# ielym/fastvision

Hardware: AMD Instinct MI355X
Metric: images/sec (640×640, bs=32/GPU) YOLOv3 train step, 1/2/4/8 MI355X (higher is better)
Workload: dtype bf16

## Files before the change

### fastvision_amd/_lib.py

```python
import ctypes as C
import os

HERE = os.path.dirname(os.path.abspath(__file__))
LIB_PATH = os.path.join(HERE, 'csrc', 'libfastvision_amd.so')
if os.environ.get('FVA_LIB_PATH'):
    if os.environ.get('FVA_EXPERIMENTS') == '1':
        LIB_PATH = os.environ['FVA_LIB_PATH']
        import sys
        print(f'fastvision_amd: EXPERIMENT -- loading {LIB_PATH} instead of the in-tree library (FVA_LIB_PATH)', file=sys.stderr)
    else:
        raise RuntimeError('fastvision_amd: FVA_LIB_PATH is set but FVA_EXPERIMENTS=1 is not -- refusing to load another library silently')

F32, BF16 = 0, 1


class ConvDesc(C.Structure):
    _fields_ = [(n, C.c_int32) for n in ('dtype', 'B', 'H', 'W', 'Cin', 'Cout', 'ksize', 'stride', 'in_pad', 'dy_pad')]


class GConvDesc(C.Structure):
    _fields_ = [(n, C.c_int32) for n in ('dtype', 'B', 'H', 'W', 'C', 'groups', 'stride', 'in_pad', 'dy_pad')]


class HeadLevel(C.Structure):
# ... 60 lines not shown
class ColourJob(C.Structure):
    _fields_ = [(n, C.c_int32) for n in ('h', 'w', 'clahe', 'hsv', 'blur')] + [('perm', C.c_int32 * 3)]


class MatchOut(C.Structure):
    _fields_ = [(n, C.c_void_p) for n in ('count', 'b', 'gx', 'gy', 'a', 'cls', 'xywh', 'anc')]


_P, _I, _L, _F = C.c_void_p, C.c_int32, C.c_int64, C.c_float
_D = C.POINTER(ConvDesc)
_H = C.POINTER(HeadLevel)
_G = C.POINTER(GConvDesc)

PROTOTYPES = {
    'fva_last_error': (C.c_char_p, []),
    'fva_version': (_I, []),
    'fva_profile_start': (_I, [_I]),
    'fva_profile_classes': (_I, [C.c_uint32, _I]),
    'fva_side_stream_fork': (_I, [_P, C.POINTER(C.c_void_p)]),
    'fva_side_stream_join': (_I, [_P]),
    'fva_side_stream_renew': (_I, []),
    'fva_conv_debug_stamps': (_I, [_P, _I]),
    'fva_conv_patch_kernel': (_I, [_I]),
    'fva_profile_stop': (_I, [_P, _P, _P, _I]),
    'fva_conv_pack_weights': (_I, [_D, _P, _P, _P, _P]),
    'fva_conv_packed_elems': (_L, [_D, _I]),
    'fva_conv_pack_weights_multi': (_I, [_P, _I, _L, _P]),
    'fva_conv_pack_weights_tiled': (_I, [_P, _I, _I, _P]),
    'fva_conv_last_kernel': (C.c_char_p, []),
    'fva_conv_fwd': (_I, [_D, _P, _P, _P, _P, _P]),
    'fva_conv1x1_fwd_apply': (_I, [_D, _P, _P, _P, _P, _I, _P, _P, _P, _P, _P]),
    'fva_conv_fwd_acc': (_I, [_D, _P, _P, _P, _P, _I, _P]),
    'fva_bn_acc_finalize': (_I, [C.POINTER(BnFwdAcc), _L, _I, _P]),
    'fva_bn_silu_apply_acc': (_I, [_I, _P, C.POINTER(BnFwdAcc), _P, _I, _P, _I, _I, _I, _I, _I, _P]),
    'fva_conv1x1_fwd_apply_acc': (_I, [_D, _P, C.POINTER(BnFwdAcc), _P, _I, _P, _P, _P, _P, _I, _P]),
    'fva_conv_fwd_bnact': (_I, [_D, _P, _P, _P, _P, _P, _P, _I, _P]),
    'fva_conv_stat_blocks': (_I, [_D]),
    'fva_conv_dgrad': (_I, [_D, _P, _P, _P, _P, _P]),
    'fva_conv_dgrad_bnstats': (_I, [_D, _P, _P, _P, _P, C.POINTER(BnBwdFuse), _P]),
    'fva_conv_dgrad_stat_rows': (_I, [_D]),
    'fva_conv_wgrad': (_I, [_D, _P, _P, _P, _I, _P, _L, _P]),
    'fva_conv_wgrad_workspace': (_L, [_D]),
    'fva_conv_wgrad_plan': (_I, [_I]),
    'fva_stem_fwd': (_I, [_I, _P, _P, _P, _P, _P, _L, _I, _I, _I, _I, _I, _P]),
    'fva_stem_fwd_workspace': (_L, [_I, _I, _I, _I]),
    'fva_stem_stat_blocks': (_I, [_I, _I, _I, _I]),
# ... 86 lines not shown
    'fva_bn_frozen_bwd_blocks': (_I, [_I, _I, _I, _I, _I, _I]),
    'fva_bn_silu_frozen_bwd': (_I, [_I, _P, _P, _P, _P, _P, _P, _P, _P, _I, _I, _I, _I, _I, _P]),
    'fva_bn_relu_frozen_bwd': (_I, [_I, _P, _P, _P, _P, _P, _P, _P, _P, _I, _I, _I, _I, _I, _P]),
    'fva_bn_frozen_bwd_finalize': (_I, [_P, _I, _I, _I, _P, _P, _P, _P, _P]),
    'fva_bn_frozen_stats': (_I, [_I, _P, _P, _P, _F, _P, _P, _P]),
    'fva_stem7_kp': (_I, [_I, _I]),
    'fva_stem7_patches': (_I, [_I, _P, _P, _I, _I, _I, _I, _P]),
    'fva_maxpool3s2_fwd': (_I, [_I, _P, _I, _P, _I, _I, _I, _I, _I, _P]),
    'fva_maxpool3s2_bwd': (_I, [_I, _P, _P, _I, _P, _I, _I, _I, _I, _P]),
    'fva_subsample2_fwd': (_I, [_I, _P, _I, _P, _I, _I, _I, _I, _P]),
    'fva_subsample2_bwd': (_I, [_I, _P, _P, _I, _I, _I, _I, _P]),
    'fva_bn_add_relu_apply': (_I, [_I, _P, _P, _P, _P, _I, _P, _P, _P, _P, _I, _I, _I, _I, _I, _P]),
    'fva_bn_add_relu_bwd_blocks': (_I, [_I, _L, _I]),
    'fva_bn_add_relu_bwd_reduce': (_I, [_I, _P, _P, _P, _P, _P, _P, _P, _I, _P, _P, _P, _P, _P, _P, _P, _I, _I, _I, _I, _I, _P]),
    'fva_bn_add_relu_bwd_apply': (_I, [_I, _P, _P, _P, _P, _P, _P, _P, _P, _I, _P, _P, _P, _P, _P, _P, _P, _P, _I, _P, _I, _I, _I, _I, _P]),
    'fva_gconv_fwd': (_I, [_G, _P, _P, _P, _P, _P]),
    'fva_gconv_stat_blocks': (_I, [_G]),
    'fva_gconv_dgrad': (_I, [_G, _P, _P, _P, _P]),
    'fva_gconv_wgrad': (_I, [_G, _P, _P, _P, _P, _L, _P]),
    'fva_gconv_wgrad_workspace': (_L, [_G]),
}
LABEL_I64, LABEL_F32 = 0, 1
REDUCE_MEAN, REDUCE_SUM = 0, 1
UNCHECKED = {'fva_conv_patch_kernel', 'fva_sgd_chunk_elems', 'fva_ema_chunk_elems', 'fva_rows_relu_bwd_rows', 'fva_colour_workspace', 'fva_conv_dgrad_stat_rows', 'fva_bias_relu_bwd_rows', 'fva_colsum_scratch_rows', 'fva_last_error', 'fva_version', 'fva_profile_stop', 'fva_conv_last_kernel', 'fva_conv_packed_elems', 'fva_conv_stat_blocks', 'fva_conv_wgrad_workspace', 'fva_conv_wgrad_plan',
             'fva_stem_stat_blocks', 'fva_stem_fused_blocks', 'fva_stem_wgrad_workspace', 'fva_stem_fwd_workspace', 'fva_stem_wgrad_mfma_workspace', 'fva_bn_bwd_blocks', 'fva_bn_partial_rows', 'fva_yolov3_loss_workspace',
             'fva_demo_loss_workspace', 'fva_demo_ciou_loss_workspace', 'fva_nms_candidates_workspace', 'fva_nms_select_workspace', 'fva_softmax_ce_workspace', 'fva_bn_frozen_bwd_blocks', 'fva_stem7_kp', 'fva_bn_add_relu_bwd_blocks', 'fva_gconv_stat_blocks', 'fva_gconv_wgrad_workspace'}

_lib = None


def load():
    global _lib
    if _lib is not None:
        return _lib
    if not os.path.exists(LIB_PATH):
        raise RuntimeError(f'fastvision_amd: {LIB_PATH} is missing -- the HIP extension is REQUIRED (no CPU fallback). '
                           'Build it with `python fastvision_amd/csrc/build.py`.')
    lib = C.CDLL(LIB_PATH)
    for name, (res, args) in PROTOTYPES.items():
        fn = getattr(lib, name)
        fn.restype, fn.argtypes = res, args
    _lib = lib
    return lib


tracer = None

# ... 22 lines not shown
```

### fastvision_amd/csrc/conv_igemm.hip

```cpp
#include <stddef.h>
#include <stdlib.h>

#include "common.h"

namespace {

enum { EPI_STATS = 0, EPI_PLAIN = 1, EPI_HEAD = 2, EPI_BNACT = 3, EPI_BNB = 4 };
constexpr int MAX_TAPS = 10;

struct IgemmParams {
    const void* in;
    const void* wt;
    void* out;
    float* stats;
    int acc_rep, bnb_rep, ax_rep;
    long long* stats_acc;
    const float* bias;
    const float* scale;
    int act;
    const float* shift;
    int M, N, C;
    int OW, OHW;
    FastDiv div_ow, div_ohw;
    int in_img, in_row;
    int sy, sx, y0, x0;
    int ktiles, kt_per_tap, halfrow;
    int ktaps;
    int tap_pix[MAX_TAPS];
    int tap_w[MAX_TAPS];
    int out_dense;
    int out_img, out_row, osy, osx, ooy, oox, out_pitch;
    const void* addend;
    int nblocks;
    const void* bnb_y;
    const float *bnb_scale, *bnb_shift, *bnb_mean, *bnb_rstd;
    float* bnb_part;
    long long* bnb_acc;
    int bnb_row0, bnb_C;
    const void* ax_y;
    const void* ax_res;
    void* ax_z;
    const float *ax_scale, *ax_shift;
    int ax_pad, ax_res_pad, ax_H, ax_W;
    long long* ax_acc;
    long long* ax_zero;
    const float *ax_gamma, *ax_beta;
    float *ax_rm, *ax_rv;
    long long* ax_nbt;
    float ax_momentum, ax_eps;
    BnN ax_n;
    float *ax_save_mean, *ax_save_rstd, *ax_scale_out, *ax_shift_out;
    long long* stamps;
    int stamp_rows;
    int pt_tx, pt_ty, pt_H, pt_W;
    int pt_tiles, pt_tpb;
    FastDiv pt_div_tx, pt_div_img;
// ... 177 lines not shown
#pragma unroll
    for (int mt = 0; mt < 4; ++mt)
#pragma unroll
        for (int nt = 0; nt < 4; ++nt)
#pragma unroll
            for (int j = 0; j < 4; ++j) f(mt * 16 + r, nt * 16 + g * 4 + j, nt, acc.a[mt][nt][j]);
}
template <typename F>
__device__ __forceinline__ void foreach_acc(Acc<float>& acc, int lane, F&& f) {
    const int r = lane & 31, h = lane >> 5;
#pragma unroll
    for (int mt = 0; mt < 2; ++mt)
#pragma unroll
        for (int nt = 0; nt < 2; ++nt)
#pragma unroll
            for (int e = 0; e < 16; ++e) f(mt * 32 + (e & 3) + 8 * (e >> 2) + 4 * h, nt * 32 + r, nt, acc.a[mt][nt][e]);
}

template <int N>
__device__ __forceinline__ void wait_vmcnt() {
    asm volatile("s_waitcnt vmcnt(%0)" ::"n"(N) : "memory");
}

template <typename T, int BM, int BN, int EPI, int NSTAGE, bool AX = false>
__global__ __launch_bounds__((BM / 64) * (BN / 64) * 64) void igemm_kernel(const IgemmParams p) {
    static_assert(!AX || (sizeof(T) == 2 && EPI == EPI_STATS), "the produced-operand form is the bf16 training forward of a 1x1 layer");
    constexpr int EPC = 16 / (int)sizeof(T);
    constexpr int BK = 8 * EPC;
    constexpr int WN = BN / 64;
    constexpr int NW = (BM / 64) * WN;
    constexpr int NT = NW * 64;
    static_assert(NW % 2 == 0, "the source swizzle assumes an even wave count");
    constexpr int A_BYTES = BM * 128, B_BYTES = BN * 128, STAGE = A_BYTES + B_BYTES;
    constexpr int A_ITERS = BM / (8 * NW), B_ITERS = BN / (8 * NW);
    constexpr bool IS_BF16 = sizeof(T) == 2;
    extern __shared__ __attribute__((aligned(16))) char smem[];

    const int tid = threadIdx.x, lane = tid & 63, w = tid >> 6;
    const int wr = w / WN, wc = w % WN;
    auto stamp = [&](int i) {
        if (p.stamps && tid == 0 && (int)blockIdx.x < p.stamp_rows) p.stamps[(int64_t)blockIdx.x * 8 + i] = wall_clock64();
    };
    stamp(0);

    const int nwg = gridDim.x, bid = blockIdx.x;
    const int xcd = bid & 7, xq = nwg >> 3, xr = nwg & 7;
    const int logical = (xcd < xr ? xcd * (xq + 1) : xr * (xq + 1) + (xcd - xr) * xq) + (bid >> 3);
    const int mblk = logical / p.nblocks, nblk = logical - mblk * p.nblocks;
    const int m0 = mblk * BM, n0 = nblk * BN;

    const T* a_ptr[A_ITERS];
    const T* b_ptr[B_ITERS];
    const int lrow = lane >> 3;
    const int sw = ((w & 1) << 2) + (lane >> 4);
    const int chunk = (lane & 7) ^ sw;
    const int tapsel = chunk >> 2;
    const int sub = p.halfrow ? (chunk & 3) : chunk;
#pragma unroll
    for (int i = 0; i < A_ITERS; ++i) {
        int m = m0 + (i * NW + w) * 8 + lrow;
        m = m < p.M ? m : p.M - 1;
        const uint32_t b = fd_div((uint32_t)m, p.div_ohw);
        const uint32_t rem = (uint32_t)m - b * (uint32_t)p.OHW;
        const uint32_t oy = fd_div(rem, p.div_ow);
        const uint32_t ox = rem - oy * (uint32_t)p.OW;
        const int64_t pix = (int64_t)b * p.in_img + (int64_t)(oy * p.sy + p.y0) * p.in_row + (ox * p.sx + p.x0);
        a_ptr[i] = (const T*)p.in + pix * p.C + sub * EPC;
    }
#pragma unroll
    for (int i = 0; i < B_ITERS; ++i) {
        int n = n0 + (i * NW + w) * 8 + lrow;
        n = n < p.N ? n : p.N - 1;
        b_ptr[i] = (const T*)p.wt + (int64_t)n * p.C + sub * EPC;
    }

    constexpr bool USE_KTAB = BN >= 128;
    constexpr int COEF_BYTES = (EPI == EPI_BNB && IS_BF16 && BN >= 128) ? 4 * BN * 4 : 0;
    float* coef_tab = (float*)(smem + NSTAGE * STAGE);
    int* ktab = (int*)(smem + NSTAGE * STAGE + COEF_BYTES);
    constexpr int COEF_PER_THREAD = COEF_BYTES > 0 ? 4 * BN / NT : 0;
    float coef_v[COEF_PER_THREAD > 0 ? COEF_PER_THREAD : 1];
    if constexpr (COEF_BYTES > 0) {
#pragma unroll
        for (int j = 0; j < COEF_PER_THREAD; ++j) coef_v[j] = bnb_coef_at<BN, NT>(p, tid + j * NT, n0);
    }
    if constexpr (USE_KTAB) {
        const int nent = p.halfrow ? 2 * p.ktiles : p.ktiles;
        for (int e = tid; e < nent; e += NT) {
            int t, kk;
            if (p.halfrow) { t = e; kk = 0; }
            else if (p.ktaps) { kk = e / p.ktaps; t = e - kk * p.ktaps; }
            else { t = e / p.kt_per_tap; kk = e - t * p.kt_per_tap; }
            int tp = 0, tw = 0;
#pragma unroll
            for (int i = 0; i < MAX_TAPS; ++i)
                if (i == t) { tp = p.tap_pix[i]; tw = p.tap_w[i]; }
            ktab[2 * e] = tp * p.C + kk * BK;
            ktab[2 * e + 1] = tw * p.N * p.C + kk * BK;
        }
        __syncthreads();
    }
    stamp(6);
    int ld_tap = 0, ld_kk = 0;
    auto load_tile = [&](int kt, int stage) {
        char* sA = smem + stage * STAGE;
        char* sB = sA + A_BYTES;
        int aoff, boff;
        if constexpr (USE_KTAB) {
            const int e = p.halfrow ? 2 * kt + tapsel : kt;
            aoff = ktab[2 * e];
            boff = ktab[2 * e + 1];
        } else {
            const int t = p.halfrow ? ld_tap + tapsel : ld_tap;
            int tp = 0, tw = 0;
#pragma unroll
// ... 10 lines not shown
#pragma unroll
        for (int i = 0; i < B_ITERS; ++i)
            __builtin_amdgcn_global_load_lds(GLB_PTR(b_ptr[i] + boff), LDS_PTR(sB + (i * NW + w) * 1024), 16, 0, 0);
    };

    bf16x8 y_pre[8], a_pre[8];
    constexpr bool PREFETCH = (EPI == EPI_BNB || EPI == EPI_PLAIN) && sizeof(T) == 2;
    if constexpr (PREFETCH) {
        constexpr int CPR = BN / 8, RSTEP = NT / CPR;
        static_assert(BM * CPR / NT == 8, "the prefetch covers the whole store loop");
        const int cc = tid % CPR, r0 = tid / CPR;
        const int n = n0 + cc * 8;
#pragma unroll
        for (int j = 0; j < 8; ++j) {
            const int m = m0 + r0 + j * RSTEP;
            int64_t oi = 0;
            if (n < p.N && m < p.M) {
                int64_t pixel = m;
                if (!p.out_dense) {
                    const uint32_t b = fd_div((uint32_t)m, p.div_ohw);
                    const uint32_t rem = (uint32_t)m - b * (uint32_t)p.OHW;
                    const uint32_t oy = fd_div(rem, p.div_ow);
                    const uint32_t ox = rem - oy * (uint32_t)p.OW;
                    pixel = (int64_t)b * p.out_img + (int64_t)(oy * p.osy + p.ooy) * p.out_row + (ox * p.osx + p.oox);
                }
                oi = pixel * p.out_pitch + n;
            }
            if constexpr (EPI == EPI_BNB) y_pre[j] = ld_stream((const bf16_t*)p.bnb_y + oi);
            if (p.addend != nullptr) a_pre[j] = ld_stream((const bf16_t*)p.addend + oi);
        }
    }

    Acc<T> acc;
    if constexpr (sizeof(T) == 2) {
#pragma unroll
        for (int i = 0; i < 4; ++i)
#pragma unroll
            for (int j = 0; j < 4; ++j) acc.a[i][j] = f32x4{0.f, 0.f, 0.f, 0.f};
    } else {
#pragma unroll
        for (int i = 0; i < 2; ++i)
#pragma unroll
            for (int j = 0; j < 2; ++j)
#pragma unroll
                for (int e = 0; e < 16; ++e) acc.a[i][j][e] = 0.f;
    }

// ... 131 lines not shown
            m = live ? m : p.M - 1;
            const uint32_t b = fd_div((uint32_t)m, p.div_ohw);
            const uint32_t rem = (uint32_t)m - b * (uint32_t)p.OHW;
            const uint32_t oy = fd_div(rem, p.div_ow);
            const uint32_t ox = rem - oy * (uint32_t)p.OW;
            ax_yo[i] = (uint32_t)m * (uint32_t)p.C + chunk * 8;
            ax_zo[i] = (b * zHW + (oy + zp) * zW + ox + zp) * (uint32_t)p.C + chunk * 8;
            ax_ro[i] = (b * rHW + (oy + rp) * rW + ox + rp) * (uint32_t)p.C + chunk * 8;
            ax_fl[i] = (live ? 1u : 0u) | (zp > 0 && live ? ((ox == 0 ? 2u : 0u) | (ox == (uint32_t)p.ax_W - 1 ? 4u : 0u) | (oy == 0 ? 8u : 0u) |
                                                           (oy == (uint32_t)p.ax_H - 1 ? 16u : 0u)) : 0u);
        }
        ax_load_raw(0, std::integral_constant<int, 0>{});
        if constexpr (AXT) {
            for (int c = tid; c < p.C; c += NT) ax_coef(c, logical == 0, ax_tab[c], ax_tab[p.C + c]);
            __syncthreads();
        }
        if (AXT && p.ax_acc != nullptr && logical == 0) {
            if (tid == 0 && p.ax_nbt) *p.ax_nbt += 1;
            fx_zero(p.ax_zero, p.C, p.ax_rep, tid, NT);
        }
        ax_issue_b(0, 0);
    } else {
        load_tile(0, 0);
        if (p.ktiles > 1) load_tile(1, 1);
    }
    stamp(1);
    for (int kt = 0; kt < p.ktiles; ++kt) {
        if constexpr (AX) {
            if (AXS == 1 || (kt & 1) == 0) ax_step(kt, std::integral_constant<int, 0>{});
            else ax_step(kt, std::integral_constant<int, AXS - 1>{});
            if (kt == 0) stamp(2);
        } else {
        if (kt == 0 && p.ktiles > 1) wait_vmcnt<LPT>();
        else wait_vmcnt<0>();
        __builtin_amdgcn_s_barrier();
        if (kt == 0) stamp(2);
        if (kt >= 1 && kt + 1 < p.ktiles) load_tile(kt + 1, st_cur ^ 1);
        }
        const char* sA = smem + st_cur * STAGE;
        const char* sB = sA + A_BYTES;
        st_cur ^= 1;
        if constexpr (IS_BF16) {
            const int r = lane & 15, g = lane >> 4, sr = (r >> 1) & 7;
            const char* pa = sA + (wr * 64 + r) * 128;
            const char* pb = sB + (wc * 64 + r) * 128;
#pragma unroll
            for (int ks = 0; ks < 2; ++ks) {
                const int co = ((ks * 4 + g) ^ sr) << 4;
                bf16x8 af[4], bfr[4];
#pragma unroll
                for (int t = 0; t < 4; ++t) {
                    af[t] = *(const bf16x8*)(pa + t * 16 * 128 + co);
                    bfr[t] = *(const bf16x8*)(pb + t * 16 * 128 + co);
                }
#pragma unroll
                for (int mt = 0; mt < 4; ++mt)
#pragma unroll
                    for (int nt = 0; nt < 4; ++nt)
                        acc.a[mt][nt] = __builtin_amdgcn_mfma_f32_16x16x32_bf16(bfr[nt], af[mt], acc.a[mt][nt], 0, 0, 0);
            }
// ... 95 lines not shown
                }
                __syncthreads();
                if (w < BN / 32) {
                    const int which = lane >> 5, col = w * 32 + (lane & 31);
                    float s = 0.f;
#pragma unroll
                    for (int k = 0; k < WMc; ++k) s += red[(which * WMc + k) * BN + col];
                    if (n0 + col < p.N) {
                        if (p.stats_acc != nullptr) fx_atomic_add(fx_replica(p.stats_acc, p.N, p.acc_rep), p.N, which, n0 + col, s);
                        else *(p.stats + ((int64_t)mblk * 2 + which) * p.N + n0 + col) = s;
                    }
                }
                __syncthreads();
            }
        }
    }

    auto out_pixel = [&](int m) -> int64_t {
        if (p.out_dense) return m;
        const uint32_t b = fd_div((uint32_t)m, p.div_ohw);
        const uint32_t rem = (uint32_t)m - b * (uint32_t)p.OHW;
        const uint32_t oy = fd_div(rem, p.div_ow);
        const uint32_t ox = rem - oy * (uint32_t)p.OW;
        return (int64_t)b * p.out_img + (int64_t)(oy * p.osy + p.ooy) * p.out_row + (ox * p.osx + p.oox);
    };

    if constexpr (EPI == EPI_HEAD) {
        float* out = (float*)p.out;
        foreach_acc(acc, lane, [&](int row, int col, int, float v) {
            const int m = m0 + wrow0 + row, n = n0 + wcol0 + col;
            if (m < p.M && n < p.N) out[(int64_t)m * p.out_pitch + n] = v + p.bias[n];
        });
    } else if constexpr (!IS_BF16) {
        float* out = (float*)p.out;
        int64_t pix_cache = -1;
        int m_cache = -1;
        constexpr bool bnb = EPI == EPI_BNB;
        float b1[2] = {0.f, 0.f}, b2[2] = {0.f, 0.f}, ksc[2], ksh[2], kmu[2], krs[2];
        if constexpr (bnb) {
#pragma unroll
            for (int nt = 0; nt < 2; ++nt) {
                int c = n0 + wcol0 + nt * 32 + (lane & 31);
                c = c < p.N ? c : p.N - 1;
                c = c >= p.bnb_C ? c - p.bnb_C : c;
                ksc[nt] = p.bnb_scale[c]; ksh[nt] = p.bnb_shift[c]; kmu[nt] = p.bnb_mean[c]; krs[nt] = p.bnb_rstd[c];
            }
        }
// ... 54 lines not shown
            static_assert(4 * BN <= NT || EPI != EPI_BNB || COEF_BYTES > 0, "one table entry per thread");
            if (tid < 4 * BN) coef_v[0] = bnb_coef_at<BN, NT>(p, tid, n0);
        }
        {
            const int r = lane & 15, g = lane >> 4;
#pragma unroll
            for (int mt = 0; mt < 4; ++mt)
#pragma unroll
                for (int nt = 0; nt < 4; ++nt) {
                    f32x4 v = acc.a[mt][nt];
                    const int col = wcol0 + nt * 16 + 4 * g;
                    if constexpr (EPI == EPI_BNACT) {
#pragma unroll
                        for (int j = 0; j < 4; ++j) v[j] = bnact_f(p, v[j], n0 + col + j < p.N ? n0 + col + j : p.N - 1);
                    }
                    *(u32x2*)(smem + (wrow0 + mt * 16 + r) * PITCH + col * 2) = u32x2{cvt_pk_bf16(v[0], v[1]), cvt_pk_bf16(v[2], v[3])};
                }
        }
        if constexpr (EPI == EPI_BNB && COEF_BYTES == 0) {
            if (tid < 4 * BN) coef_tab[tid] = coef_v[0];
        }
        __syncthreads();
        stamp(4);
        store_tile_bf16<EPI, BM, BN, NT, PITCH>(p, smem, tid, n0, mblk, [&](int row) { const int m = m0 + row; return m < p.M ? out_pixel(m) : (int64_t)-1; },
                                                EPI == EPI_BNB ? y_pre : nullptr, PREFETCH ? a_pre : nullptr, coef_tab);
    }
    stamp(5);
}

template <typename T, int BM, int BN, int EPI, int NSTAGE, bool AX = false>
int launch_one(const IgemmParams& p, hipStream_t s) {
    const int mblocks = cdiv(p.M, BM);
    IgemmParams q = p;
    q.nblocks = cdiv(p.N, BN);
    static const bool stamp_tiles = [] { const char* e = getenv("FVA_STAMP_IGEMM"); return e && atoi(e) != 0; }();
    q.stamps = stamp_tiles ? fva_debug_stamps_ptr() : nullptr;
    q.stamp_rows = stamp_tiles ? fva_debug_stamps_rows() : 0;
    constexpr int KTAB_MAX = 16384;
    const int nent = (p.halfrow ? 2 : 1) * p.ktiles;
    if (BN >= 128 && nent * 8 > KTAB_MAX) return fva_fail(FVA_ERR_ARG, "igemm: %d k-tiles exceed the offset table (%d)", p.ktiles, KTAB_MAX / 8);
    const int ktab_bytes = BN >= 128 ? (nent * 8 > 4096 ? (nent * 8 + 255) & ~255 : 4096) : 0;
    constexpr int coef_bytes = (EPI == EPI_BNB && sizeof(T) == 2 && BN >= 128) ? 4 * BN * 4 : 0;
    const int smem = NSTAGE * (BM + BN) * 128 + ktab_bytes + coef_bytes;
    static bool attr_done = false;
    if (!attr_done) {
        (void)hipFuncSetAttribute((const void*)igemm_kernel<T, BM, BN, EPI, NSTAGE, AX>, hipFuncAttributeMaxDynamicSharedMemorySize,
                                  NSTAGE * (BM + BN) * 128 + (BN >= 128 ? KTAB_MAX : 0) + coef_bytes);
        attr_done = true;
    }
    hipLaunchKernelGGL((igemm_kernel<T, BM, BN, EPI, NSTAGE, AX>), dim3(mblocks * q.nblocks), dim3((BM / 64) * (BN / 64) * 64), smem, s, q);
    FVA_LAUNCH_CHECK("igemm_kernel");
    fva_note_kernel(AX ? (BM == 128 ? "igemm128ax" : "igemm256x64ax") : (BM == 128 ? "igemm128" : "igemm256x64"));
    return FVA_OK;
}

// ... 322 lines not shown
#define FVA_EPI_STAMPS 0
#endif
template <int EPI>
__global__ __launch_bounds__(512) void igemm8_kernel(const IgemmParams p, const Igemm8Diag sk) {
    constexpr int MT = 8;
    constexpr int WM = 16 * MT;
    constexpr int BM = 2 * WM, BN = 256, NT = 512, BK = 64;
    constexpr int HALF = 128 * 128, BUF = 4 * HALF;
    constexpr int EPI_BYTES = BM * (BN * 2 + 16);
    constexpr int TAB0 = EPI_BYTES > 2 * BUF ? EPI_BYTES : 2 * BUF;
    extern __shared__ __attribute__((aligned(16))) char smem[];
    const int tid = threadIdx.x, lane = tid & 63, w = tid >> 6;
    const int wr = w >> 2, wc = w & 3;
    auto stamp = [&](int i) {
        if (sk.stamps && tid == 0 && (int)blockIdx.x < sk.stamp_rows) {
            sk.stamps[(int64_t)blockIdx.x * 8 + i] = wall_clock64();
            sk.stamps[(int64_t)blockIdx.x * 8 + 4 + i] = clock64();
        }
    };
#if !FVA_EPI_STAMPS
    stamp(0);
#endif

    const int nwg = gridDim.x, bid = blockIdx.x;
    const int xcd = bid & 7, xq = nwg >> 3, xr = nwg & 7;
    const int logical = (xcd < xr ? xcd * (xq + 1) : xr * (xq + 1) + (xcd - xr) * xq) + (bid >> 3);
    const int KT = p.ktiles;

    int* ktab = (int*)(smem + TAB0);
    for (int e = tid; e < KT; e += NT) {
        int t, kk;
        if (p.ktaps) { kk = e / p.ktaps; t = e - kk * p.ktaps; }
        else { t = e / p.kt_per_tap; kk = e - t * p.kt_per_tap; }
        int tp = 0, tw = 0;
#pragma unroll
        for (int i = 0; i < MAX_TAPS; ++i)
            if (i == t) { tp = p.tap_pix[i]; tw = p.tap_w[i]; }
        ktab[2 * e] = tp * p.C + kk * BK;
        ktab[2 * e + 1] = tw * p.N * p.C + kk * BK;
    }

    const int lrow = lane >> 3;
    const int chunk = (lane & 7) ^ (((w & 1) << 2) + (lane >> 4));
    const int r = lane & 15, g = lane >> 4, sr = (r >> 1) & 7;
    const int co0 = (g ^ sr) << 4, co1 = ((4 + g) ^ sr) << 4;
    const int a_row = (wr * 64 + r) * 128, b_row = (wc * 32 + r) * 128;

    {
        const int tile = logical, kt0 = 0, kt1 = KT;
        const int mblk = tile / p.nblocks, nblk = tile - mblk * p.nblocks;
        const int m0 = mblk * BM, n0 = nblk * BN;
        __syncthreads();
        float* coef_tab = (float*)(smem + TAB0 + 4096);
        if constexpr (EPI == EPI_BNB) bnb_fill_lds<BN, NT>(p, coef_tab, tid, n0);

        uint32_t a_off[2][2], b_off[2][2];
// ... 156 lines not shown
                    *(f32x4*)(red + ((1 * 2 + wr_e) * 16 + r_e) * RP + col_e + ni * 16) = s2[ni];
                }
                __syncthreads();
                {
                    const int which = lane_e >> 5, col = (tid_e >> 6) * 32 + (lane_e & 31);
                    float s = 0.f;
#pragma unroll
                    for (int i = 0; i < 32; ++i) s += red[(which * 32 + i) * RP + col];
                    if (n0 + col < p.N) {
                        if (p.stats_acc != nullptr) fx_atomic_add(fx_replica(p.stats_acc, p.N, p.acc_rep), p.N, which, n0 + col, s);
                        else *(p.stats + ((int64_t)mblk * 2 + which) * p.N + n0 + col) = s;
                    }
                }
                __syncthreads();
            }
        }

        auto out_pixel = [&](int m) -> int64_t {
            if (p.out_dense) return m;
            const uint32_t b = fd_div((uint32_t)m, p.div_ohw);
            const uint32_t rem = (uint32_t)m - b * (uint32_t)p.OHW;
            const uint32_t oy = fd_div(rem, p.div_ow);
            const uint32_t ox = rem - oy * (uint32_t)p.OW;
            return (int64_t)b * p.out_img + (int64_t)(oy * p.osy + p.ooy) * p.out_row + (ox * p.osx + p.oox);
        };
        constexpr int PITCH = BN * 2 + 16;
#if FVA_EPI_STAMPS
        stamp(1);
#endif
#pragma unroll
        for (int mi = 0; mi < MT; ++mi)
#pragma unroll
            for (int ni = 0; ni < 4; ++ni) {
                f32x4 v = acc[mi][ni];
                if constexpr (EPI == EPI_BNACT) {
#pragma unroll
                    for (int j = 0; j < 4; ++j) v[j] = bnact_f(p, v[j], n0 + col_e + ni * 16 + j);
                }
                *(u32x2*)(smem + (row_e + mi * 16) * PITCH + (col_e + ni * 16) * 2) = u32x2{cvt_pk_bf16(v[0], v[1]), cvt_pk_bf16(v[2], v[3])};
            }
        __syncthreads();
#if FVA_EPI_STAMPS
        stamp(2);
#endif
        store_tile_bf16<EPI, BM, BN, NT, PITCH>(p, smem, tid_e, n0, mblk, [&](int row) { const int m = m0 + row; return m < p.M ? out_pixel(m) : (int64_t)-1; },
                                                nullptr, nullptr, EPI == EPI_BNB ? coef_tab : nullptr);
    }
    stamp(3);
}

constexpr int IGEMM8_SMEM = 256 * (256 * 2 + 16) + 4096 + 4096;

inline bool igemm8_enabled() {
    static bool v = [] {
        const char* e = getenv("FVA_IGEMM8");
        return !e || atoi(e) != 0;
    }();
    return v;
}
inline bool use_igemm8(int dtype, int64_t M, int N, int C, int ntaps, int64_t in_pixels) {
    if (!igemm8_enabled() || dtype != FVA_BF16 || N % 256 || C % 64) return false;
    if (in_pixels * C * 2 >= (1ll << 31) || (int64_t)(ntaps + 1) * N * C * 2 >= (1ll << 31)) return false;
    const int64_t ktiles = (int64_t)ntaps * (C / 64), tiles = (int64_t)cdiv(M, 256) * (N / 256);
    if (ktiles > 496 || ktiles < 8) return false;
    if (tiles < 128) return false;
    static const int min_kt = [] { const char* e = getenv("FVA_IGEMM8_MINKT"); return e ? atoi(e) : 16; }();
    return ktiles >= min_kt || tiles <= 256;
}

long long* g_stamps = nullptr;
int g_stamp_rows = 0;

template <int EPI>
int launch_igemm8(const IgemmParams& p, hipStream_t s) {
    IgemmParams q = p;
    q.nblocks = p.N / 256;
    const int tiles = cdiv(p.M, 256) * q.nblocks;
    static bool attr_done = false;
    if (!attr_done) {
        (void)hipFuncSetAttribute((const void*)igemm8_kernel<EPI>, hipFuncAttributeMaxDynamicSharedMemorySize, IGEMM8_SMEM);
        attr_done = true;
    }
    Igemm8Diag sk{};
    sk.stamps = g_stamps;
    sk.stamp_rows = g_stamp_rows;
    hipLaunchKernelGGL((igemm8_kernel<EPI>), dim3(tiles), dim3(512), IGEMM8_SMEM, s, q, sk);
    fva_note_kernel("igemm8");
    FVA_LAUNCH_CHECK("igemm8_kernel");
    return FVA_OK;
}

inline bool wide_tile(int N) { return N >= 128; }

enum { IGEMM_128, IGEMM_256x64, IGEMM_8PHASE };
struct IgemmChoice {
    int kernel, bm;
};
inline IgemmChoice choose_igemm(int dtype, int64_t M, int N, int C, int ntaps, int64_t in_pixels, bool halfrow, bool head) {
    if (!head && !halfrow && use_igemm8(dtype, M, N, C, ntaps, in_pixels)) return {IGEMM_8PHASE, 256};
    return wide_tile(N) ? IgemmChoice{IGEMM_128, 128} : IgemmChoice{IGEMM_256x64, 256};
// ... 198 lines not shown
}
inline bool dgrad_paired(int dtype, int ksize, int stride, int Cin, int Cout) {
    return ksize == 3 && stride == 2 && Cin <= pair_max_cin() && !use_pdgrad2(dtype, ksize, stride, Cout, Cin);
}

int packed_taps(const fva_conv_desc* d, int for_dgrad) {
    if (for_dgrad && dgrad_paired(d->dtype, d->ksize, d->stride, d->Cin, d->Cout)) return 12;

    const int kk = d->ksize * d->ksize;
    const int C = for_dgrad ? d->Cout : d->Cin;
    return (halfrow_mode(d->dtype, C) && (kk & 1)) ? kk + 1 : kk;
}

enum { LAUNCH_IGEMM, LAUNCH_PATCH1, LAUNCH_PATCH2 };
struct ConvLaunch {
    int kind;
    IgemmChoice igemm;
    int64_t M;
    int N, OH, OW;
    int ntaps, tap_pix[MAX_TAPS], tap_w[MAX_TAPS];
    int ostep, ooy, oox;
    int row_blocks;
    int rows_per_block;
};

void set_grid(ConvLaunch& e, int B, int OH, int OW, int N) {
    e.M = (int64_t)B * OH * OW; e.N = N; e.OH = OH; e.OW = OW;
    e.ntaps = 0; e.ostep = 1; e.ooy = e.oox = 0; e.rows_per_block = 1;
}
void add_tap(ConvLaunch& e, int pix, int w) { e.tap_pix[e.ntaps] = pix; e.tap_w[e.ntaps] = w; ++e.ntaps; }
void close_taps(ConvLaunch& e, int zero_tap) { e.tap_w[e.ntaps] = zero_tap; }
void finish_igemm(ConvLaunch& e, int dtype, int C, int64_t in_pixels, bool head) {
    e.kind = LAUNCH_IGEMM;
    e.igemm = choose_igemm(dtype, e.M, e.N, C, e.ntaps, in_pixels, halfrow_mode(dtype, C), head);
    e.row_blocks = cdiv(e.M, e.igemm.bm);
}
template <typename G>
void finish_patch(ConvLaunch& e, int kind, const fva_conv_desc* d) {
    e.kind = kind;
    e.row_blocks = patch_tiles<G>(d->B, d->H, d->W);
}

ConvLaunch fwd_plan(const fva_conv_desc* d, int epi) {
    const int k = d->ksize, s = d->stride, in_row = d->W + 2 * d->in_pad, in_img = (d->H + 2 * d->in_pad) * in_row;
    ConvLaunch e;
    set_grid(e, d->B, (d->H - 1) / s + 1, (d->W - 1) / s + 1, d->Cout);
    if (k * k < MAX_TAPS) {
        for (int kh = 0; kh < k; ++kh)
            for (int kw = 0; kw < k; ++kw) add_tap(e, kh * in_row + kw, kh * k + kw);
        close_taps(e, k * k);
    } else {
        e.ntaps = k * k;
    }
    finish_igemm(e, d->dtype, d->Cin, (int64_t)(d->B + 1) * in_img, epi == EPI_HEAD);
    if (epi == EPI_STATS && use_pconv(d->dtype, k, s, d->Cin, d->Cout, d->H, d->W)) finish_patch<PconvGeom>(e, LAUNCH_PATCH1, d);
    return e;
}

int parity_taps(int parity, int kh[2], int off[2]) {
    if (parity == 0) { kh[0] = 1; off[0] = 0; return 1; }
    kh[0] = 0; off[0] = 1; kh[1] = 2; off[1] = 0;
    return 2;
}

int dgrad_plan(const fva_conv_desc* d, ConvLaunch out[4]) {
    const int k = d->ksize, s = d->stride, pd = k / 2, dtype = d->dtype;
    const int OH = (d->H - 1) / s + 1, OW = (d->W - 1) / s + 1, in_row = OW + 2 * d->dy_pad;
    const int64_t in_pixels = (int64_t)(d->B + 1) * (OH + 2 * d->dy_pad) * in_row;
    ConvLaunch& e = out[0];
    if (s == 1) {
        set_grid(e, d->B, d->H, d->W, d->Cin);
        for (int kh = 0; kh < k; ++kh)
            for (int kw = 0; kw < k; ++kw) add_tap(e, (2 * pd - kh) * in_row + (2 * pd - kw), kh * k + kw);
        close_taps(e, k * k);
        finish_igemm(e, dtype, d->Cout, in_pixels, false);
        if (use_pconv(dtype, k, s, d->Cout, d->Cin, d->H, d->W)) finish_patch<PconvGeom>(e, LAUNCH_PATCH1, d);
        return 1;
    }
    if (use_pdgrad2(dtype, k, s, d->Cout, d->Cin)) {
        set_grid(e, d->B, d->H, d->W, d->Cin);
        finish_patch<Pdgrad2Geom>(e, LAUNCH_PATCH2, d);
        return 1;
    }
    const bool paired = dgrad_paired(dtype, k, s, d->Cin, d->Cout);
    int n = 0;
    for (int py = 0; py < 2; ++py)
        for (int px = 0; px < (paired ? 1 : 2); ++px) {
            ConvLaunch& q = out[n++];
            set_grid(q, d->B, d->H / 2, d->W / 2, paired ? 2 * d->Cin : d->Cin);
            int ky[2], yo[2], kx[2] = {0, 1}, xo[2] = {0, 1};
            const int ny = parity_taps(py, ky, yo), nx = paired ? 2 : parity_taps(px, kx, xo);
            for (int a = 0; a < ny; ++a)
                for (int b = 0; b < nx; ++b) add_tap(q, (d->dy_pad + yo[a]) * in_row + d->dy_pad + xo[b], ky[a] * (paired ? 2 : 3) + kx[b]);
            q.ostep = 2; q.ooy = py; q.oox = px;
            q.rows_per_block = paired ? 2 : 1;
            close_taps(q, paired ? 0 : 9);
            finish_igemm(q, dtype, d->Cout, in_pixels, false);
        }
    return n;
}

}

long long* fva_debug_stamps_ptr() { return g_stamps; }
int fva_debug_stamps_rows() { return g_stamp_rows; }
extern "C" {

int fva_conv_patch_kernel(int on) {
    const int prev = pconv_enabled() ? 1 : 0;
    g_pconv = on ? 1 : 0;
    return prev;
}

int fva_conv_debug_stamps(void* stamps, int32_t rows) {
    if (stamps && rows < 1) return fva_fail(FVA_ERR_ARG, "fva_conv_debug_stamps: rows must be >= 1");
    g_stamps = (long long*)stamps;
    g_stamp_rows = stamps ? rows : 0;
    return FVA_OK;
}

int64_t fva_conv_packed_elems(const fva_conv_desc* d, int for_dgrad) {
    if (!d) return 0;
    return (int64_t)packed_taps(d, for_dgrad) * d->Cout * d->Cin;
}

int fva_conv_pack_weights(const fva_conv_desc* d, const float* w, void* w_fwd, void* w_dgrad, void* stream) {
    int rc = check_desc(d, "fva_conv_pack_weights");
    if (rc) return rc;
    if (!w) return fva_fail(FVA_ERR_ARG, "fva_conv_pack_weights: null weights");
    const int paired = dgrad_paired(d->dtype, d->ksize, d->stride, d->Cin, d->Cout) ? 1 : 0;
    const int tf = packed_taps(d, 0), td = paired ? d->ksize * d->ksize : packed_taps(d, 1);
    const int64_t total = (int64_t)(tf > td ? tf : td) * d->Cout * d->Cin;
    const int grid = (int)((total + 255) / 256 < 4096 ? (total + 255) / 256 : 4096);
// ... 18 lines not shown
    hipLaunchKernelGGL(pack_weights_tiled_kernel, dim3(total_tiles), dim3(256), 0, (hipStream_t)stream, table_dev, n);
    FVA_LAUNCH_CHECK("pack_weights_tiled_kernel");
    return FVA_OK;
}

int32_t fva_conv_stat_blocks(const fva_conv_desc* d) {
    if (!d) return 0;
    return fwd_plan(d, EPI_STATS).row_blocks;
}

static void set_launch(IgemmParams& p, const ConvLaunch& e, int dtype) {
    p.M = (int)e.M;
    p.N = e.N;
    p.OW = e.OW;
    p.OHW = e.OH * e.OW;
    p.div_ow = make_fastdiv(p.OW);
    p.div_ohw = make_fastdiv(p.OHW);
    for (int t = 0; t < e.ntaps; ++t) {
        p.tap_pix[t] = e.tap_pix[t];
        p.tap_w[t] = e.tap_w[t];
    }
    p.tap_w[e.ntaps] = e.tap_w[e.ntaps];
    finish_taps(p, e.ntaps, dtype);
    p.out_dense = e.ostep == 1 ? 1 : 0;
    if (!p.out_dense) {
        p.osy = p.osx = e.ostep;
        p.ooy = e.ooy;
        p.oox = e.oox;
    }
}

static int setup_fwd(const fva_conv_desc* d, int epi, IgemmParams& p, ConvLaunch& e, const char* who) {
    int rc = check_desc(d, who);
    if (rc) return rc;
    rc = check_red_channels(d->dtype, d->Cin, who);
    if (rc) return rc;
    e = fwd_plan(d, epi);
    p = IgemmParams();
    p.acc_rep = p.bnb_rep = p.ax_rep = 1;
    p.C = d->Cin;
    p.in_row = d->W + 2 * d->in_pad;
    p.in_img = (d->H + 2 * d->in_pad) * p.in_row;
    p.sy = p.sx = d->stride;
    p.y0 = p.x0 = d->in_pad - d->ksize / 2;
    set_launch(p, e, d->dtype);
    p.out_pitch = d->Cout;
// ... 214 lines not shown
```

### include/fastvision_amd.h

```cpp
#ifndef FASTVISION_AMD_H
#define FASTVISION_AMD_H

#include <stdint.h>

#ifdef __cplusplus
extern "C" {
#endif

typedef enum { FVA_F32 = 0, FVA_BF16 = 1 } fva_dtype;

typedef enum {
    FVA_OK = 0,
    FVA_ERR_ARG = -1,
    FVA_ERR_LAUNCH = -2,
    FVA_ERR_WORKSPACE = -3
} fva_status;

const char* fva_last_error(void);
int fva_version(void);

int fva_profile_start(int32_t max_spans);
int fva_profile_classes(uint32_t mask, int32_t stride);

int fva_side_stream_fork(void* main_stream, void** side_stream);
// ... 7 lines not shown
    int32_t Cin, Cout;
    int32_t ksize, stride;
    int32_t in_pad;
    int32_t dy_pad;
} fva_conv_desc;

int fva_conv_pack_weights(const fva_conv_desc* d, const float* w_oihw, void* w_fwd, void* w_dgrad, void* stream);
int64_t fva_conv_packed_elems(const fva_conv_desc* d, int for_dgrad);
typedef struct {
    const float* w;
    void* w_fwd;
    void* w_dgrad;
    int32_t Cout, Cin, ksize, taps_fwd, taps_dgrad, dtype;
    int32_t dgrad_paired;
    int32_t tile_start;
} fva_pack_entry;
int fva_conv_pack_weights_multi(const fva_pack_entry* table, int32_t n, int64_t max_elems, void* stream);
int fva_conv_pack_weights_tiled(const fva_pack_entry* table, int32_t n, int32_t total_tiles, void* stream);

const char* fva_conv_last_kernel(void);

int fva_conv_debug_stamps(void* stamps, int32_t rows);
int fva_conv_patch_kernel(int on);

int fva_conv_fwd(const fva_conv_desc* d, const void* x, const void* w_fwd, void* y, float* stats_partial, void* stream);
int fva_conv1x1_fwd_apply(const fva_conv_desc* d, const void* y_prev, const float* scale, const float* shift, const void* residual,
                          int32_t res_pad, void* z, const void* w_fwd, void* y, float* stats_partial, void* stream);
int fva_conv_fwd_bnact(const fva_conv_desc* d, const void* x, const void* w_fwd, const float* scale, const float* shift,
                       const void* residual, void* z, int32_t z_pad, void* stream);
int32_t fva_conv_stat_blocks(const fva_conv_desc* d);

int fva_conv_dgrad(const fva_conv_desc* d, const void* dy, const void* w_dgrad, void* dx, const void* addend, void* stream);

typedef struct {
    const void* y;
    const float *scale, *shift, *mean, *rstd;
    float* partial;
    int64_t* acc;
    int32_t acc_replicas;
} fva_bn_bwd_fuse;
int fva_conv_dgrad_bnstats(const fva_conv_desc* d, const void* dy, const void* w_dgrad, void* dx, const void* addend,
                           const fva_bn_bwd_fuse* fuse, void* stream);
int32_t fva_conv_dgrad_stat_rows(const fva_conv_desc* d);

int fva_conv_wgrad(const fva_conv_desc* d, const void* x, const void* dy, float* dw_oihw, int accumulate,
                   void* workspace, int64_t workspace_bytes, void* stream);
// ... 300 lines not shown
```

Baseline: 1130.

## Merge four stride-2 dgrad parity classes into a single igemm launch

The data-gradient of stride-2 convolutions was computed as up to four separate igemm launches, one per output parity class. This merges them into one grid: each block decodes its parity class from its block index using a small per-class descriptor (tap offset, tap count, output offset, stat block base). Heavier classes are ordered first, and the tile size is re-chosen for the merged problem. The aim is to remove launch overhead and the tail underutilisation of small per-class grids. The cost is extra index arithmetic in both igemm kernels, and the merge is on by default with an env var and API toggle to turn it off.

```diff
diff --git a/fastvision_amd/_lib.py b/fastvision_amd/_lib.py
--- a/fastvision_amd/_lib.py
+++ b/fastvision_amd/_lib.py
@@ -106,6 +106,7 @@
     'fva_side_stream_renew': (_I, []),
     'fva_conv_debug_stamps': (_I, [_P, _I]),
     'fva_conv_patch_kernel': (_I, [_I]),
+    'fva_conv_dgrad_merge': (_I, [_I]),
     'fva_profile_stop': (_I, [_P, _P, _P, _I]),
     'fva_conv_pack_weights': (_I, [_D, _P, _P, _P, _P]),
     'fva_conv_packed_elems': (_L, [_D, _I]),
@@ -238,7 +239,7 @@
 }
 LABEL_I64, LABEL_F32 = 0, 1
 REDUCE_MEAN, REDUCE_SUM = 0, 1
-UNCHECKED = {'fva_conv_patch_kernel', 'fva_sgd_chunk_elems', 'fva_ema_chunk_elems', 'fva_rows_relu_bwd_rows', 'fva_colour_workspace', 'fva_conv_dgrad_stat_rows', 'fva_bias_relu_bwd_rows', 'fva_colsum_scratch_rows', 'fva_last_error', 'fva_version', 'fva_profile_stop', 'fva_conv_last_kernel', 'fva_conv_packed_elems', 'fva_conv_stat_blocks', 'fva_conv_wgrad_workspace', 'fva_conv_wgrad_plan',
+UNCHECKED = {'fva_conv_patch_kernel', 'fva_conv_dgrad_merge', 'fva_sgd_chunk_elems', 'fva_ema_chunk_elems', 'fva_rows_relu_bwd_rows', 'fva_colour_workspace', 'fva_conv_dgrad_stat_rows', 'fva_bias_relu_bwd_rows', 'fva_colsum_scratch_rows', 'fva_last_error', 'fva_version', 'fva_profile_stop', 'fva_conv_last_kernel', 'fva_conv_packed_elems', 'fva_conv_stat_blocks', 'fva_conv_wgrad_workspace', 'fva_conv_wgrad_plan',
              'fva_stem_stat_blocks', 'fva_stem_fused_blocks', 'fva_stem_wgrad_workspace', 'fva_stem_fwd_workspace', 'fva_stem_wgrad_mfma_workspace', 'fva_bn_bwd_blocks', 'fva_bn_partial_rows', 'fva_yolov3_loss_workspace',
              'fva_demo_loss_workspace', 'fva_demo_ciou_loss_workspace', 'fva_nms_candidates_workspace', 'fva_nms_select_workspace', 'fva_softmax_ce_workspace', 'fva_bn_frozen_bwd_blocks', 'fva_stem7_kp', 'fva_bn_add_relu_bwd_blocks', 'fva_gconv_stat_blocks', 'fva_gconv_wgrad_workspace'}
 
diff --git a/fastvision_amd/csrc/conv_igemm.hip b/fastvision_amd/csrc/conv_igemm.hip
--- a/fastvision_amd/csrc/conv_igemm.hip
+++ b/fastvision_amd/csrc/conv_igemm.hip
@@ -32,6 +32,8 @@
     int out_img, out_row, osy, osx, ooy, oox, out_pitch;
     const void* addend;
     int nblocks;
+    int cls_blocks;
+    int cls_desc[4];
     const void* bnb_y;
     const float *bnb_scale, *bnb_shift, *bnb_mean, *bnb_rstd;
     float* bnb_part;
@@ -255,6 +257,31 @@
     asm volatile("s_waitcnt vmcnt(%0)" ::"n"(N) : "memory");
 }
 
+struct TileClass {
+    int bid, nwg, ktiles, ktaps, tap0, ooy, oox, stat_blk0;
+};
+template <bool ON>
+__device__ __forceinline__ TileClass tile_class(const IgemmParams& p) {
+    TileClass c{(int)blockIdx.x, (int)gridDim.x, p.ktiles, p.ktaps, 0, p.ooy, p.oox, 0};
+    if constexpr (ON) {
+        if (p.cls_blocks) {
+            const int per = p.cls_blocks * p.nblocks;
+            const int i = (c.bid >= per ? 1 : 0) + (c.bid >= 2 * per ? 1 : 0) + (c.bid >= 3 * per ? 1 : 0);
+            const int dsc = i == 0 ? p.cls_desc[0] : i == 1 ? p.cls_desc[1] : i == 2 ? p.cls_desc[2] : p.cls_desc[3];
+            const int ntaps = (dsc >> 4) & 15;
+            c.bid -= i * per;
+            c.nwg = per;
+            c.ktiles = ntaps * p.kt_per_tap;
+            c.ktaps = p.ktaps ? ntaps : 0;
+            c.tap0 = dsc & 15;
+            c.ooy = (dsc >> 8) & 1;
+            c.oox = (dsc >> 9) & 1;
+            c.stat_blk0 = ((dsc >> 10) & 3) * p.cls_blocks;
+        }
+    }
+    return c;
+}
+
 template <typename T, int BM, int BN, int EPI, int NSTAGE, bool AX = false>
 __global__ __launch_bounds__((BM / 64) * (BN / 64) * 64) void igemm_kernel(const IgemmParams p) {
     static_assert(!AX || (sizeof(T) == 2 && EPI == EPI_STATS), "the produced-operand form is the bf16 training forward of a 1x1 layer");
@@ -276,7 +303,8 @@
     };
     stamp(0);
 
-    const int nwg = gridDim.x, bid = blockIdx.x;
+    const TileClass tc = tile_class<(EPI == EPI_PLAIN || EPI == EPI_BNB) && IS_BF16 && BM == 128 && BN == 128 && !AX>(p);
+    const int nwg = tc.nwg, bid = tc.bid;
     const int xcd = bid & 7, xq = nwg >> 3, xr = nwg & 7;
     const int logical = (xcd < xr ? xcd * (xq + 1) : xr * (xq + 1) + (xcd - xr) * xq) + (bid >> 3);
     const int mblk = logical / p.nblocks, nblk = logical - mblk * p.nblocks;
@@ -318,12 +346,13 @@
         for (int j = 0; j < COEF_PER_THREAD; ++j) coef_v[j] = bnb_coef_at<BN, NT>(p, tid + j * NT, n0);
     }
     if constexpr (USE_KTAB) {
-        const int nent = p.halfrow ? 2 * p.ktiles : p.ktiles;
+        const int nent = p.halfrow ? 2 * tc.ktiles : tc.ktiles;
         for (int e = tid; e < nent; e += NT) {
             int t, kk;
             if (p.halfrow) { t = e; kk = 0; }
-            else if (p.ktaps) { kk = e / p.ktaps; t = e - kk * p.ktaps; }
+            else if (tc.ktaps) { kk = e / tc.ktaps; t = e - kk * tc.ktaps; }
             else { t = e / p.kt_per_tap; kk = e - t * p.kt_per_tap; }
+            t += tc.tap0;
             int tp = 0, tw = 0;
 #pragma unroll
             for (int i = 0; i < MAX_TAPS; ++i)
@@ -380,7 +409,7 @@
                     const uint32_t rem = (uint32_t)m - b * (uint32_t)p.OHW;
                     const uint32_t oy = fd_div(rem, p.div_ow);
                     const uint32_t ox = rem - oy * (uint32_t)p.OW;
-                    pixel = (int64_t)b * p.out_img + (int64_t)(oy * p.osy + p.ooy) * p.out_row + (ox * p.osx + p.oox);
+                    pixel = (int64_t)b * p.out_img + (int64_t)(oy * p.osy + tc.ooy) * p.out_row + (ox * p.osx + tc.oox);
                 }
                 oi = pixel * p.out_pitch + n;
             }
@@ -558,20 +587,20 @@
         ax_issue_b(0, 0);
     } else {
         load_tile(0, 0);
-        if (p.ktiles > 1) load_tile(1, 1);
+        if (tc.ktiles > 1) load_tile(1, 1);
     }
     stamp(1);
-    for (int kt = 0; kt < p.ktiles; ++kt) {
+    for (int kt = 0; kt < tc.ktiles; ++kt) {
         if constexpr (AX) {
             if (AXS == 1 || (kt & 1) == 0) ax_step(kt, std::integral_constant<int, 0>{});
             else ax_step(kt, std::integral_constant<int, AXS - 1>{});
             if (kt == 0) stamp(2);
         } else {
-        if (kt == 0 && p.ktiles > 1) wait_vmcnt<LPT>();
+        if (kt == 0 && tc.ktiles > 1) wait_vmcnt<LPT>();
         else wait_vmcnt<0>();
         __builtin_amdgcn_s_barrier();
         if (kt == 0) stamp(2);
-        if (kt >= 1 && kt + 1 < p.ktiles) load_tile(kt + 1, st_cur ^ 1);
+        if (kt >= 1 && kt + 1 < tc.ktiles) load_tile(kt + 1, st_cur ^ 1);
         }
         const char* sA = smem + st_cur * STAGE;
         const char* sB = sA + A_BYTES;
@@ -713,7 +742,7 @@
         const uint32_t rem = (uint32_t)m - b * (uint32_t)p.OHW;
         const uint32_t oy = fd_div(rem, p.div_ow);
         const uint32_t ox = rem - oy * (uint32_t)p.OW;
-        return (int64_t)b * p.out_img + (int64_t)(oy * p.osy + p.ooy) * p.out_row + (ox * p.osx + p.oox);
+        return (int64_t)b * p.out_img + (int64_t)(oy * p.osy + tc.ooy) * p.out_row + (ox * p.osx + tc.oox);
     };
 
     if constexpr (EPI == EPI_HEAD) {
@@ -814,7 +843,7 @@
         }
         __syncthreads();
         stamp(4);
-        store_tile_bf16<EPI, BM, BN, NT, PITCH>(p, smem, tid, n0, mblk, [&](int row) { const int m = m0 + row; return m < p.M ? out_pixel(m) : (int64_t)-1; },
+        store_tile_bf16<EPI, BM, BN, NT, PITCH>(p, smem, tid, n0, tc.stat_blk0 + mblk, [&](int row) { const int m = m0 + row; return m < p.M ? out_pixel(m) : (int64_t)-1; },
                                                 EPI == EPI_BNB ? y_pre : nullptr, PREFETCH ? a_pre : nullptr, coef_tab);
     }
     stamp(5);
@@ -822,7 +851,7 @@
 
 template <typename T, int BM, int BN, int EPI, int NSTAGE, bool AX = false>
 int launch_one(const IgemmParams& p, hipStream_t s) {
-    const int mblocks = cdiv(p.M, BM);
+    const int mblocks = p.cls_blocks ? 4 * p.cls_blocks : cdiv(p.M, BM);
     IgemmParams q = p;
     q.nblocks = cdiv(p.N, BN);
     static const bool stamp_tiles = [] { const char* e = getenv("FVA_STAMP_IGEMM"); return e && atoi(e) != 0; }();
@@ -1191,16 +1220,18 @@
     stamp(0);
 #endif
 
-    const int nwg = gridDim.x, bid = blockIdx.x;
+    const TileClass tc = tile_class<EPI == EPI_PLAIN || EPI == EPI_BNB>(p);
+    const int nwg = tc.nwg, bid = tc.bid;
     const int xcd = bid & 7, xq = nwg >> 3, xr = nwg & 7;
     const int logical = (xcd < xr ? xcd * (xq + 1) : xr * (xq + 1) + (xcd - xr) * xq) + (bid >> 3);
-    const int KT = p.ktiles;
+    const int KT = tc.ktiles;
 
     int* ktab = (int*)(smem + TAB0);
     for (int e = tid; e < KT; e += NT) {
         int t, kk;
-        if (p.ktaps) { kk = e / p.ktaps; t = e - kk * p.ktaps; }
+        if (tc.ktaps) { kk = e / tc.ktaps; t = e - kk * tc.ktaps; }
         else { t = e / p.kt_per_tap; kk = e - t * p.kt_per_tap; }
+        t += tc.tap0;
         int tp = 0, tw = 0;
 #pragma unroll
         for (int i = 0; i < MAX_TAPS; ++i)
@@ -1403,7 +1434,7 @@
             const uint32_t rem = (uint32_t)m - b * (uint32_t)p.OHW;
             const uint32_t oy = fd_div(rem, p.div_ow);
             const uint32_t ox = rem - oy * (uint32_t)p.OW;
-            return (int64_t)b * p.out_img + (int64_t)(oy * p.osy + p.ooy) * p.out_row + (ox * p.osx + p.oox);
+            return (int64_t)b * p.out_img + (int64_t)(oy * p.osy + tc.ooy) * p.out_row + (ox * p.osx + tc.oox);
         };
         constexpr int PITCH = BN * 2 + 16;
 #if FVA_EPI_STAMPS
@@ -1424,7 +1455,7 @@
 #if FVA_EPI_STAMPS
         stamp(2);
 #endif
-        store_tile_bf16<EPI, BM, BN, NT, PITCH>(p, smem, tid_e, n0, mblk, [&](int row) { const int m = m0 + row; return m < p.M ? out_pixel(m) : (int64_t)-1; },
+        store_tile_bf16<EPI, BM, BN, NT, PITCH>(p, smem, tid_e, n0, tc.stat_blk0 + mblk, [&](int row) { const int m = m0 + row; return m < p.M ? out_pixel(m) : (int64_t)-1; },
                                                 nullptr, nullptr, EPI == EPI_BNB ? coef_tab : nullptr);
     }
     stamp(3);
@@ -1456,7 +1487,7 @@
 int launch_igemm8(const IgemmParams& p, hipStream_t s) {
     IgemmParams q = p;
     q.nblocks = p.N / 256;
-    const int tiles = cdiv(p.M, 256) * q.nblocks;
+    const int tiles = (p.cls_blocks ? 4 * p.cls_blocks : cdiv(p.M, 256)) * q.nblocks;
     static bool attr_done = false;
     if (!attr_done) {
         (void)hipFuncSetAttribute((const void*)igemm8_kernel<EPI>, hipFuncAttributeMaxDynamicSharedMemorySize, IGEMM8_SMEM);
@@ -1701,11 +1732,12 @@
     int ostep, ooy, oox;
     int row_blocks;
     int rows_per_block;
+    int cls_blocks, cls_desc[4];
 };
 
 void set_grid(ConvLaunch& e, int B, int OH, int OW, int N) {
     e.M = (int64_t)B * OH * OW; e.N = N; e.OH = OH; e.OW = OW;
-    e.ntaps = 0; e.ostep = 1; e.ooy = e.oox = 0; e.rows_per_block = 1;
+    e.ntaps = 0; e.ostep = 1; e.ooy = e.oox = 0; e.rows_per_block = 1; e.cls_blocks = 0;
 }
 void add_tap(ConvLaunch& e, int pix, int w) { e.tap_pix[e.ntaps] = pix; e.tap_w[e.ntaps] = w; ++e.ntaps; }
 void close_taps(ConvLaunch& e, int zero_tap) { e.tap_w[e.ntaps] = zero_tap; }
@@ -1740,6 +1772,44 @@
     if (parity == 0) { kh[0] = 1; off[0] = 0; return 1; }
     kh[0] = 0; off[0] = 1; kh[1] = 2; off[1] = 0;
     return 2;
+}
+
+int g_dgrad_merge = -1;
+inline bool dgrad_merge_enabled() {
+    if (g_dgrad_merge < 0) {
+        const char* e = getenv("FVA_DGRAD_MERGE");
+        g_dgrad_merge = (!e || atoi(e) != 0) ? 1 : 0;
+    }
+    return g_dgrad_merge != 0;
+}
+
+bool merge_parity_classes(const ConvLaunch cls[4], int dtype, int C, int64_t in_pixels, ConvLaunch& m) {
+    if (!dgrad_merge_enabled() || dtype != FVA_BF16 || halfrow_mode(dtype, C)) return false;
+    const int alone = cls[0].igemm.kernel;
+    if (alone != IGEMM_128 && alone != IGEMM_8PHASE) return false;
+    for (int c = 1; c < 4; ++c)
+        if (cls[c].igemm.kernel != alone) return false;
+    m = cls[0];
+    m.ntaps = 0;
+    int tap0[4];
+    for (int c = 0; c < 4; ++c) {
+        tap0[c] = m.ntaps;
+        for (int t = 0; t < cls[c].ntaps; ++t) add_tap(m, cls[c].tap_pix[t], cls[c].tap_w[t]);
+    }
+    close_taps(m, 9);
+    const int64_t m8 = 4 * (int64_t)cdiv(m.M, 256) * 256;
+    const bool fits32 = (int64_t)(9 + 1) * m.N * C * 2 < (1ll << 31);
+    if (alone == IGEMM_8PHASE && !fits32) return false;
+    const bool eight = alone == IGEMM_8PHASE || (fits32 && use_igemm8(dtype, m8, m.N, C, 1, in_pixels) && use_igemm8(dtype, m8, m.N, C, 4, in_pixels));
+    m.igemm = eight ? IgemmChoice{IGEMM_8PHASE, 256} : IgemmChoice{IGEMM_128, 128};
+    m.cls_blocks = cdiv(m.M, m.igemm.bm);
+    m.row_blocks = 4 * m.cls_blocks;
+    const int order[4] = {3, 1, 2, 0};
+    for (int i = 0; i < 4; ++i) {
+        const int c = order[i];
+        m.cls_desc[i] = tap0[c] | cls[c].ntaps << 4 | cls[c].ooy << 8 | cls[c].oox << 9 | c << 10;
+    }
+    return true;
 }
 
 int dgrad_plan(const fva_conv_desc* d, ConvLaunch out[4]) {
@@ -1776,6 +1846,11 @@
             close_taps(q, paired ? 0 : 9);
             finish_igemm(q, dtype, d->Cout, in_pixels, false);
         }
+    ConvLaunch merged;
+    if (!paired && merge_parity_classes(out, dtype, d->Cout, in_pixels, merged)) {
+        out[0] = merged;
+        return 1;
+    }
     return n;
 }
 
@@ -1788,6 +1863,12 @@
 int fva_conv_patch_kernel(int on) {
     const int prev = pconv_enabled() ? 1 : 0;
     g_pconv = on ? 1 : 0;
+    return prev;
+}
+
+int fva_conv_dgrad_merge(int on) {
+    const int prev = dgrad_merge_enabled() ? 1 : 0;
+    g_dgrad_merge = on ? 1 : 0;
     return prev;
 }
 
@@ -1852,6 +1933,11 @@
     }
     p.tap_w[e.ntaps] = e.tap_w[e.ntaps];
     finish_taps(p, e.ntaps, dtype);
+    p.cls_blocks = e.cls_blocks;
+    if (e.cls_blocks) {
+        for (int i = 0; i < 4; ++i) p.cls_desc[i] = e.cls_desc[i];
+        p.ktiles = 4 * p.kt_per_tap;
+    }
     p.out_dense = e.ostep == 1 ? 1 : 0;
     if (!p.out_dense) {
         p.osy = p.osx = e.ostep;
diff --git a/include/fastvision_amd.h b/include/fastvision_amd.h
--- a/include/fastvision_amd.h
+++ b/include/fastvision_amd.h
@@ -53,6 +53,7 @@
 
 int fva_conv_debug_stamps(void* stamps, int32_t rows);
 int fva_conv_patch_kernel(int on);
+int fva_conv_dgrad_merge(int on);
 
 int fva_conv_fwd(const fva_conv_desc* d, const void* x, const void* w_fwd, void* y, float* stats_partial, void* stream);
 int fva_conv1x1_fwd_apply(const fva_conv_desc* d, const void* y_prev, const float* scale, const float* shift, const void* residual,
```

Result: no change. 1136 (median of 6 runs) (+0.6%).
